# jonaselgammal/GPry

Measured on AMD Instinct MI355X. Metric: gp_refit_plus_nora_acq_cycle_throughput, higher is better.
Workload: dtype f64

## Files before the change

gpry_amd/_lib.py:

```python
import ctypes as C
import ctypes as _ct
import os

import numpy as np

_HERE = os.path.dirname(os.path.abspath(__file__))
LIB_PATH = os.path.join(_HERE, "libgpry_hip.so")

GPRY_MAX_DIM = 32
MASK_CLASSIFIED_INF = 1
MASK_OUTSIDE_TRUST = 2

KERNEL_IDS = {"rbf": 0, "matern12": 1, "matern32": 2, "matern52": 3}
KERNEL_WHITE = 0x10


class GpryAffine(C.Structure):
    _fields_ = [("has_x_affine", C.c_int),
                ("x_lo", C.c_double * GPRY_MAX_DIM),
                ("x_span", C.c_double * GPRY_MAX_DIM),
                ("y_mean", C.c_double), ("y_std", C.c_double),
                ("clip_hi", C.c_double)]


# ... 79 lines not shown
    "gpry_sweep_logexp": (C.c_int, [_vp, _vp, C.c_int64, _vp, C.c_double, C.c_double,
                                    C.c_double, _vp, _vp, _vp, _P(C.c_int64)]),
    "gpry_sweep_logexp_given": (C.c_int, [_vp, _vp, C.c_int64, _vp, _vp, _vp, C.c_double, C.c_double,
                                          C.c_double, _vp, _vp, _vp, _P(C.c_int64)]),
    "gpry_sweep_fetch": (C.c_int, [_vp, C.c_int64, _vp, _vp, _vp]),
    "gpry_sweep_prune_info": (C.c_int, [_vp, _vp, _vp]),
    "gpry_sweep_screen_info": (C.c_int, [_vp, _vp]),
    "gpry_sweep_topk": (C.c_int, [_vp, C.c_int64, _vp, C.c_int64, _vp, _P(C.c_int64),
                                  _P(C.c_double)]),
    "gpry_kb_reset": (C.c_int, [_vp]),
    "gpry_kb_register": (C.c_int, [_vp, _vp, C.c_int64, _P(C.c_int64), _vp]),
    "gpry_kb_gram": (C.c_int, [_vp, C.c_int64, _vp, _vp, _P(C.c_int64)]),
    "gpry_kb_gram_rows": (C.c_int, [_vp, _vp, C.c_int64, _vp, _vp, _P(C.c_int64)]),
    "gpry_kb_rank": (C.c_int, [_vp, _vp, C.c_int64, _vp, C.c_int64, _vp, _vp, _vp, _vp, C.c_int64, _vp, C.c_int64, _vp,
                               C.c_int64, _vp, _vp, _vp, _vp, _vp, _P(C.c_int64), _P(C.c_int64), _vp]),
    "gpry_comm_unique_id": (C.c_int, [_vp]),
    "gpry_comm_init": (C.c_int, [_vp, C.c_int, C.c_int, _vp, _P(_vp)]),
    "gpry_comm_destroy": (C.c_int, [_vp]),
    "gpry_comm_info": (C.c_int, [_vp, _P(C.c_int), _P(C.c_int), _P(C.c_int)]),
    "gpry_comm_allgather": (C.c_int, [_vp, _vp, C.c_int64, _vp]),
    "gpry_comm_allreduce_max": (C.c_int, [_vp, _vp, C.c_int64]),
    "gpry_comm_barrier": (C.c_int, [_vp]),
    "gpry_group_create": (C.c_int, [C.c_int, _P(C.c_int), _vp, _P(_vp)]),
    "gpry_group_destroy": (C.c_int, [_vp]),
    "gpry_group_size": (C.c_int, [_vp, _P(C.c_int), _P(C.c_int)]),
    "gpry_group_member": (_vp, [_vp, C.c_int]),
    "gpry_group_last_error": (C.c_char_p, [_vp]),
    "gpry_group_set_model": (C.c_int, [_vp, _vp, _vp, _vp, C.c_int64, C.c_int, C.c_int, _vp,
                                       _P(GpryAffine), _P(C.c_int)]),
    "gpry_group_set_gates": (C.c_int, [_vp, _vp, _vp, C.c_int64, C.c_double, C.c_double, C.c_int, _vp]),
# ... 819 lines not shown
        s_idx, s_y, s_sigma, s_acq, s_cond = slots
        for a, t in ((var0, np.float64), (idx, np.int64), (y, np.float64), (sigma, np.float64), (acq, np.float64),
                     (order, np.int64), (s_idx, np.int64), (s_y, np.float64), (s_sigma, np.float64),
                     (s_acq, np.float64), (s_cond, np.float64)):
            if a.dtype != t or not a.flags.c_contiguous:
                raise ValueError("kb_rank: arrays must be contiguous int64 / float64")
        if not (len(y) == len(sigma) == len(acq) == len(idx)) or len(params) != 5 or \
                not (len(s_idx) == len(s_y) == len(s_sigma) == len(s_acq) == len(s_cond)):
            raise ValueError("kb_rank: array lengths do not match")
        self._check(self._lib.gpry_kb_rank(self._h, _ptr(X_new), m_new, _ptr(var0), len(var0), _ptr(idx), _ptr(y),
                                           _ptr(sigma), _ptr(acq), len(idx), _ptr(order), len(order), _ptr(params),
                                           len(s_idx) - 1, _ptr(s_idx), _ptr(s_y), _ptr(s_sigma), _ptr(s_acq),
                                           _ptr(s_cond), C.byref(counter), C.byref(info), _ptr(stats)), "gpry_kb_rank")
        return counter.value, info.value, stats

    def timing_reset(self):
        self._check(self._lib.gpry_timing_reset(self._h), "gpry_timing_reset")

    def timing(self, name):
        ms, cnt = C.c_double(0.0), C.c_int64(0)
        self._lib.gpry_timing_get(self._h, name.encode(), C.byref(ms), C.byref(cnt))
        return ms.value, cnt.value

    def debug_gemm(self, A, B, C0, M, N, K, a_trans=False, b_trans=False, epi=0, kmode=0,
                   lower_only=False, tile_map=0):
        A, B = _f64(A), _f64(B)
        crow = (M + 127) // 128 if epi == 3 else M
        Cout = np.ascontiguousarray(np.zeros((crow, N)) if C0 is None else C0, dtype=np.float64).copy()
        self._check(self._lib.gpry_debug_gemm(self._h, _ptr(A), _ptr(B), _ptr(Cout), M, N, K,
                                              int(a_trans), int(b_trans), int(epi), int(kmode),
# ... 199 lines not shown
```

gpry_amd/csrc/api.hip:

```cpp
#include "sweep.h"
#include "kb_gram.h"
#include <algorithm>

int require_model(gpry_ctx* ctx, bool need_factor) {
    if (ctx->N <= 0) return gpry_fail(ctx, -1, "no training set (call gpry_set_train)");
    if (!ctx->have_theta) return gpry_fail(ctx, -1, "no hyperparameters (call gpry_set_theta)");
    if (need_factor && !ctx->factor_valid) return gpry_fail(ctx, -1, "model not factorised (call gpry_factorize)");
    if (need_factor && ctx->tf.has_x_affine)
        for (int k = 0; k < ctx->d; k++)
            if (!(ctx->tf.x_span[k] != 0.0) || !isfinite(ctx->tf.x_span[k]) || !isfinite(ctx->tf.x_lo[k]))
                return gpry_fail(ctx, -1, "affine map of X: span %g, offset %g in dimension %d of %d (gpry_set_affine of another model?)",
                                 ctx->tf.x_span[k], ctx->tf.x_lo[k], k, ctx->d);
    return 0;
}


static int copy_out_matrix(gpry_ctx* ctx, const double* dsrc, int64_t ld, int64_t rows, int64_t cols, double* hdst) {
    HIP_TRY(ctx, hipMemcpy2DAsync(hdst, sizeof(double) * cols, dsrc, sizeof(double) * ld,
                                  sizeof(double) * cols, rows, hipMemcpyDeviceToHost, ctx->stream));
    HIP_TRY(ctx, hipStreamSynchronize(ctx->stream));
    return 0;
}

bool panel_timed_out(int marker) { return (marker & 0xFF00) == 0x5A00; }
// ... 889 lines not shown
    for (int off = 32; off >= 1; off >>= 1) s += __shfl_xor(s, off);
    if (lane == 0) out[x] = C - s;
}

extern "C" {

int gpry_kb_reset(gpry_ctx* ctx) {
    if (!ctx) return gpry_fail(nullptr, -1, "gpry_kb_reset: ctx is NULL");
    GPRY_TRY(require_model(ctx, true));
    ctx->kb_n = 0;
    return 0;
}

int gpry_kb_register(gpry_ctx* ctx, const double* X, int64_t m, int64_t* first, double* var0) {
    if (!ctx) return gpry_fail(nullptr, -1, "gpry_kb_register: ctx is NULL");
    GPRY_TRY(serve_stop(ctx));
    GPRY_TRY(require_model(ctx, true));
    HIP_TRY(ctx, hipSetDevice(ctx->device));
    if (m <= 0) { if (first) *first = ctx->kb_n; return 0; }
    StageScope kb_scope(ctx, "kb_register");
    hipStream_t st = ctx->stream;
    const int64_t Np = ctx->Np;
    int64_t need = ctx->kb_n + round_up(m, 128);
    if (ctx->kb_n > 0 && ctx->kb_ld < Np) return gpry_fail(ctx, -4, "kb_register: session rows have stride %lld, model needs %lld", (long long)ctx->kb_ld, (long long)Np);
    if (need > ctx->kb_cap || Np > ctx->kb_ld) {
        int64_t cap = std::max<int64_t>(need, std::max<int64_t>(1024, need > ctx->kb_cap ? 2 * ctx->kb_cap : ctx->kb_cap));
        double *nU = nullptr, *nX = nullptr, *nO = nullptr;
        GPRY_TRY(dev_alloc(ctx, &nU, cap * Np));
        GPRY_TRY(dev_alloc(ctx, &nX, cap * ctx->dpad));
        GPRY_TRY(dev_alloc(ctx, &nO, 2 * cap));
        if (ctx->kb_n > 0) {
            HIP_TRY(ctx, hipMemcpyAsync(nU, ctx->dU, sizeof(double) * ctx->kb_n * Np, hipMemcpyDeviceToDevice, st));
            HIP_TRY(ctx, hipMemcpyAsync(nX, ctx->dXkb, sizeof(double) * ctx->kb_n * ctx->dpad, hipMemcpyDeviceToDevice, st));
        }
        HIP_TRY(ctx, hipStreamSynchronize(st));
        if (ctx->dU) GPRY_TRY(dev_free(ctx, ctx->dU));
        if (ctx->dXkb) GPRY_TRY(dev_free(ctx, ctx->dXkb));
        if (ctx->dkbout) GPRY_TRY(dev_free(ctx, ctx->dkbout));
        ctx->dU = nU; ctx->dXkb = nX; ctx->dkbout = nO; ctx->kb_cap = cap; ctx->kb_ld = Np;
    }
    const int64_t mp = round_up(m, 128);
    TmpBuf<double> bX, bpar;
    GPRY_TRY(bX.alloc(ctx, m * ctx->d));
    GPRY_TRY(bpar.alloc(ctx, 3 * GPRY_MAX_DIM));
    double *dX = bX.p, *dpar = bpar.p;
    HIP_TRY(ctx, hipMemcpyAsync(dX, X, sizeof(double) * m * ctx->d, hipMemcpyHostToDevice, st));
    double hpar[3 * GPRY_MAX_DIM];
    for (int k = 0; k < GPRY_MAX_DIM; k++) {
        hpar[k] = k < ctx->d ? ctx->tf.x_lo[k] : 0.0;
        hpar[GPRY_MAX_DIM + k] = k < ctx->d ? ctx->tf.x_span[k] : 1.0;
        hpar[2 * GPRY_MAX_DIM + k] = k < ctx->d ? exp(ctx->theta[1 + k]) : 1.0;
    }
    HIP_TRY(ctx, hipMemcpyAsync(dpar, hpar, sizeof(hpar), hipMemcpyHostToDevice, st));
    hipLaunchKernelGGL(scale_rows_kernel, dim3((unsigned)((m * ctx->dpad + 255) / 256)), dim3(256), 0, st, dX, m,
                       ctx->d, ctx->dpad, ctx->tf.has_x_affine, dpar, dpar + GPRY_MAX_DIM, dpar + 2 * GPRY_MAX_DIM,
                       ctx->dXkb + ctx->kb_n * ctx->dpad);
    GPRY_TRY(dev_grow(ctx, &ctx->dKst, &ctx->kst_cap, Np * mp));
    int64_t saveM = ctx->sw_M; ctx->sw_M = m;
    int rc = mp <= 512 ? launch_cross_build_small(ctx, dX, 0, mp, mp, ctx->dKst, nullptr, 1)
                       : launch_cross_build(ctx, dX, 0, mp, mp, ctx->dKst, nullptr, 1);
    ctx->sw_M = saveM;
// ... 1 lines not shown
    GemmArgs g = {};
    g.A = ctx->dKst; g.lda = mp;
    g.B = ctx->dV; g.ldb = Np;
    g.C = ctx->dU + ctx->kb_n * Np; g.ldc = Np;
    g.M = (int)mp; g.N = (int)Np; g.K = (int)Np;
    g.kmode = KM_B_UPPER; g.lower_only = 0; g.tile_map = TM_ROWMAJOR;
    {
        int ns = 1;
        while (ns < 8 && Np / (ns * 2) >= 256) ns *= 2;
        if (ns > 1) {
            GPRY_TRY(gemm_split_scratch(ctx, ns, mp * Np, &g.split_buf));
            g.nsplit = ns; g.split_stride = mp * Np;
        }
    }
    GPRY_TRY(gemm_f64_launch(ctx, g, true, true, EPI_STORE));
    if (var0) {
        hipLaunchKernelGGL(kb_var0_kernel, dim3((unsigned)((m + 3) / 4)), dim3(256), 0, st, ctx->dU, Np, ctx->kb_n, m,
                           Np, ctx_prior_var(ctx), ctx->dkbout);
        HIP_TRY(ctx, hipMemcpyAsync(var0, ctx->dkbout, sizeof(double) * m, hipMemcpyDeviceToHost, st));
    }
    HIP_TRY(ctx, hipStreamSynchronize(st));
    if (first) *first = ctx->kb_n;
    ctx->kb_n += m;
    return 0;
}

int gpry_kb_gram(gpry_ctx* ctx, int64_t p, double* G, double* kvec, int64_t* n) {
    if (!ctx) return gpry_fail(nullptr, -1, "gpry_kb_gram: ctx is NULL");
    GPRY_TRY(require_model(ctx, true));
    HIP_TRY(ctx, hipSetDevice(ctx->device));
    if (p < 0 || p >= ctx->kb_n) return gpry_fail(ctx, -1, "kb_gram: index %lld out of range [0, %lld)", (long long)p, (long long)ctx->kb_n);
    StageScope kb_scope(ctx, "kb_gram");
    hipStream_t st = ctx->stream;
    int64_t nn = ctx->kb_n;
    GPRY_TRY(ensure_pinned(ctx, (int64_t)sizeof(double) * 2 * nn));
    double* hres = static_cast<double*>(ctx->hpin);
    double* dres = static_cast<double*>(ctx->hpin_dev);
    hipLaunchKernelGGL(kb_gram_kernel, dim3((unsigned)((nn + 3) / 4)), dim3(256), 0, st, ctx->dU, ctx->Np, nn, p,
                       ctx->Np, ctx->dXkb, ctx->dpad, ctx->kernel_id, exp(ctx->theta[0]), dres, dres + nn);
    HIP_TRY(ctx, hipGetLastError());
// ... 76 lines not shown
```

gpry_amd/csrc/common.h:

```cpp
#pragma once
#include <hip/hip_runtime.h>
#include <stdint.h>
#include <stdio.h>
#include <string.h>
#include <math.h>
#include <string>
#include <vector>
#include <map>

#include "../../include/gpry_hip.h"

#define GPRY_THETA_MAX (2 + GPRY_MAX_DIM)
#define GPRY_BPAR_ROW (2 + GPRY_MAX_DIM)
#define GPRY_BPAR_WHITE (1 + GPRY_MAX_DIM)
#define GPRY_TILE 128
#define GPRY_NB 64

typedef double v4d __attribute__((ext_vector_type(4)));

struct StageTimer {
    double total_ms = 0.0;
    int64_t count = 0;
    std::vector<std::pair<hipEvent_t, hipEvent_t>> pending;
};
// ... 116 lines not shown
    unsigned long long* dsel = nullptr;
    enum { DSEL_NAN = 0,
           DSEL_STATE = 0,
           DSEL_EMIT = 4,
           DSEL_SURV = 6,
           DSEL_GIDX = 7,
           DSEL_LIVE = 8,
           DSEL_FALL = 9,
           DSEL_WORDS = 64 };

    int64_t kb_n = 0, kb_cap = 0;
    int64_t kb_ld = 0;
    double* dU = nullptr;
    double* dXkb = nullptr;
    double* dkbout = nullptr;

    double* dbord = nullptr;
    int64_t bord_cap = 0;
    int64_t n_border = 0;

    void* trtri_plan = nullptr;
    void* trtri_pipe = nullptr;
    int64_t opt_gemm_streamk = 5632;
    int64_t opt_topk_host = 16384;
    int opt_factor_pipeline = 1;
    int opt_factor_pipeline_min = 1280;
    void* chol_plan = nullptr;

    void* srv = nullptr;
    int opt_predict_serve = 1;
// ... 311 lines not shown
```

gpry_amd/csrc/ctx.hip:

```cpp
#include "common.h"
#include <string>
#include <stdarg.h>
#include <dlfcn.h>

thread_local char g_last_error[1024] = {0};
void trtri_plan_free(gpry_ctx* ctx);
void overlap_plan_free(gpry_ctx* ctx);

int gpry_fail(gpry_ctx* ctx, int code, const char* fmt, ...) {
    va_list ap;
    va_start(ap, fmt);
    vsnprintf(g_last_error, sizeof(g_last_error), fmt, ap);
    va_end(ap);
    if (ctx) { strncpy(ctx->err, g_last_error, sizeof(ctx->err) - 1); }
    return code;
}

template <typename T>
int dev_alloc(gpry_ctx* ctx, T** p, int64_t count) {
    *p = nullptr;
    if (count <= 0) count = 1;
    HIP_TRY(ctx, hipMalloc((void**)p, sizeof(T) * (size_t)count));
    return 0;
}
// ... 200 lines not shown
    (void)hipSetDevice(ctx->device);
    (void)hipStreamSynchronize(ctx->stream);
    if (ctx->stream2) (void)hipStreamSynchronize(ctx->stream2);
    timers_collect(ctx);
    serve_free(ctx);
    trtri_plan_free(ctx);
    trtri_pipe_free(ctx);
    overlap_plan_free(ctx);
    void* bufs[] = {ctx->dX, ctx->dXs, ctx->dy, ctx->dnoise, ctx->dA, ctx->dV, ctx->dW, ctx->dW2, ctx->dW3,
                    ctx->dalpha_, ctx->dvec, ctx->dinfo, ctx->dparams, ctx->dXc, ctx->dmask, ctx->dy_all,
                    ctx->dsig_all, ctx->dacq_all, ctx->dKst, ctx->dpart, ctx->dkeys, ctx->dhist, ctx->dselp,
                    ctx->dcand, ctx->dsel, ctx->dU, ctx->dXkb, ctx->dkbout, ctx->pr.dXc, ctx->pr.dmask,
                    ctx->pr.dy, ctx->pr.dsig, ctx->pr.dacq, ctx->dG,
                    ctx->gate_sv, ctx->gate_coef, ctx->gate_trust, ctx->dsplit, ctx->dbord, ctx->barena, ctx->dXcs, ctx->dYcs,
                    ctx->dub, ctx->dXg, ctx->dgidx, ctx->snap.dV, ctx->snap.dalpha_, ctx->snap.dXs, ctx->snap.dX, ctx->dmc, ctx->dknn,
                    ctx->dph, ctx->djoint, ctx->dloo, ctx->dsvm, ctx->dhess, ctx->dtg, ctx->dpw};
    for (void* b : bufs) if (b) (void)hipFree(b);
    if (ctx->hpin) (void)hipHostFree(ctx->hpin);
    if (ctx->hloo) (void)hipHostFree(ctx->hloo);
    if (ctx->hsvm) (void)hipHostFree(ctx->hsvm);
    if (ctx->hbres) (void)hipHostFree(ctx->hbres);
    (void)hipStreamDestroy(ctx->stream);
    if (ctx->stream2) (void)hipStreamDestroy(ctx->stream2);
    for (hipEvent_t ev : ctx->ev_pool) (void)hipEventDestroy(ev);
    for (hipStream_t st : ctx->tp_streams) (void)hipStreamDestroy(st);
    for (hipEvent_t ev : ctx->tp_events) (void)hipEventDestroy(ev);
    delete ctx;
    return 0;
}

const char* gpry_last_error(gpry_ctx* ctx) { return ctx ? ctx->err : g_last_error; }
// ... 44 lines not shown
    OPT_INT("sweep_upload", opt_sweep_upload, 0, 1, (void)0),
    OPT_INT("sweep_overlap", opt_sweep_overlap, 0, 1, (void)0),
    OPT_INT("sweep_prune", opt_sweep_prune, 0, 1, (void)0),
    OPT_INT("sweep_mean_bound", opt_sweep_mean_bound, 0, 1, (void)0),
    OPT_INT("sweep_screen", opt_sweep_screen, 0, 1, (void)0),
    OPT_INT("sweep_small_map", opt_sweep_small_map, 0, 1, (void)0),
    OPT_INT("select_fused", opt_select_fused, 0, 1, (void)0),
    OPT_INT("prune_one_select", opt_prune_one_select, 0, 1, (void)0),
    OPT_INT("chol_stacked", opt_chol_stacked, 0, BIG, c->lml_cache = false),
    OPT_INT("chol_stacked_dense", opt_chol_stacked_dense, 0, 1, c->lml_cache = false),
    OPT_INT("predict_gates", opt_predict_gates, 0, 1, (void)0),
    OPT_INT("predict_serve", opt_predict_serve, 0, 1, (void)0),
    OPT_INT("serve_idle_us", opt_serve_idle_us, 10, 1000000, (void)0),
    OPT_INT("mcmc_mapped", opt_mcmc_mapped, 0, 1, (void)0),
    OPT_INT("kb_rank", opt_kb_rank, 0, 1, (void)0),
    OPT_INT("svm_iters_per_launch", opt_svm_iters, 1, BIG, (void)0),
};
#undef OPT_INT
const OptionSpec* find_option(const char* key) {
    for (const OptionSpec& o : OPTIONS) if (!strcmp(o.key, key)) return &o;
    return nullptr;
}
}

int gpry_ctx_set_option(gpry_ctx* ctx, const char* key, int64_t value) {
    if (!ctx || !key) return gpry_fail(ctx, -1, "gpry_ctx_set_option: NULL argument");
    GPRY_TRY(serve_stop(ctx));
    const OptionSpec* o = find_option(key);
    if (!o) return gpry_fail(ctx, -1, "unknown option '%s'", key);
    if (value < o->lo || value > o->hi)
// ... 374 lines not shown
```

gpry_amd/csrc/kb_rank.hip:

```cpp
#include "common.h"
#include "kb_gram.h"
#include "kb_rank_core.h"
#include <memory>

#define KB_ROWS_MAX 64
struct KbRowList { int64_t p[KB_ROWS_MAX]; };

__global__ __launch_bounds__(256) void kb_gram_rows_kernel(const double* __restrict__ U, int64_t ldu, int64_t n, KbRowList rows,
                                                           int64_t Np, const double* __restrict__ Xkb, int dpad, int kid,
                                                           double C, double* __restrict__ out) {
    const int64_t x = (int64_t)blockIdx.x * 4 + (threadIdx.x >> 6);
    if (x >= n) return;
    double* o = out + (int64_t)blockIdx.y * 2 * n;
    kb_gram_entry(U, ldu, x, rows.p[blockIdx.y], Np, Xkb, dpad, kid, C, o, o + n);
}

namespace {
struct RowServer {
    gpry_ctx* ctx;
    int64_t nn;
    std::vector<const double*> G, kv;
    std::vector<std::unique_ptr<double[]>> store;
    int64_t launches = 0, rows = 0;

// ... 16 lines not shown
                               static_cast<double*>(ctx->hpin_dev));
            HIP_TRY(ctx, hipGetLastError());
            HIP_TRY(ctx, hipStreamSynchronize(ctx->stream));
            store.emplace_back(new double[(size_t)len]);
            double* blk = store.back().get();
            memcpy(blk, ctx->hpin, sizeof(double) * (size_t)len);
            for (int j = 0; j < cnt; j++) { G[rl.p[j]] = blk + (size_t)j * 2 * nn; kv[rl.p[j]] = blk + (size_t)j * 2 * nn + nn; }
            launches++; rows += cnt;
        }
        return 0;
    }
    static int fetch_cb(void* user, const int64_t* p, int n) { return static_cast<RowServer*>(user)->fetch(p, n); }
};
}

extern "C" {

int gpry_kb_gram_rows(gpry_ctx* ctx, const int64_t* p, int64_t n_rows, double* G, double* kvec, int64_t* n) {
    if (!ctx) return gpry_fail(nullptr, -1, "gpry_kb_gram_rows: ctx is NULL");
    GPRY_TRY(require_model(ctx, true));
    HIP_TRY(ctx, hipSetDevice(ctx->device));
    if (!p || !G || !kvec || n_rows <= 0 || n_rows > 16384) return gpry_fail(ctx, -1, "kb_gram_rows: bad arguments");
    if (ctx->kb_n <= 0) return gpry_fail(ctx, -1, "kb_gram_rows: no registered candidates");
    StageScope kb_scope(ctx, "kb_rank");
    RowServer rs{ctx, ctx->kb_n};
    rs.G.assign((size_t)rs.nn, nullptr); rs.kv.assign((size_t)rs.nn, nullptr);
    GPRY_TRY(rs.fetch(p, (int)n_rows));
    for (int64_t j = 0; j < n_rows; j++) {
        memcpy(G + j * rs.nn, rs.G[p[j]], sizeof(double) * rs.nn);
        memcpy(kvec + j * rs.nn, rs.kv[p[j]], sizeof(double) * rs.nn);
// ... 23 lines not shown
        if (ctx->kb_n + m_new != n_session)
            return gpry_fail(ctx, -1, "kb_rank: session has %lld candidates, %lld new rows, caller expects %lld",
                             (long long)ctx->kb_n, (long long)m_new, (long long)n_session);
        GPRY_TRY(gpry_kb_register(ctx, X_new, m_new, &first, var0 + (n_session - m_new)));
    }
    if (ctx->kb_n != n_session)
        return gpry_fail(ctx, -1, "kb_rank: session has %lld candidates, caller expects %lld", (long long)ctx->kb_n, (long long)n_session);
    for (int64_t i = 0; i < n_offer; i++)
        if (idx[i] < 0 || idx[i] >= n_session) return gpry_fail(ctx, -1, "kb_rank: offer %lld has session index %lld", (long long)i, (long long)idx[i]);
    for (int64_t k = 0; k < n_order; k++)
        if (order[k] < 0 || order[k] >= n_offer) return gpry_fail(ctx, -1, "kb_rank: order[%lld] = %lld", (long long)k, (long long)order[k]);
    const int n = (int)n_points;
    for (int t = 0; t <= n; t++)
        if (slot_idx[t] >= n_session || (slot_idx[t] < 0 && slot_acq_cond[t] > -INFINITY))
            return gpry_fail(ctx, -1, "kb_rank: slot %d has session index %lld", t, (long long)slot_idx[t]);
    StageScope kb_scope(ctx, "kb_rank");
    RowServer rs{ctx, n_session};
    rs.G.assign((size_t)n_session, nullptr); rs.kv.assign((size_t)n_session, nullptr);
    {
        std::vector<int64_t> spec;
        for (int t = 0; t < n; t++) if (slot_idx[t] >= 0 && slot_acq_cond[t] > -INFINITY) spec.push_back(slot_idx[t]);
        for (int64_t k = 0; k < n_order && k < 2 * (int64_t)n; k++) spec.push_back(idx[order[k]]);
        if (!spec.empty()) GPRY_TRY(rs.fetch(spec.data(), (int)spec.size()));
    }
    kb_rank::Params prm = {params[0], params[1], params[2], params[3], params[4]};
    kb_rank::Pool P = {n, slot_idx, slot_y, slot_sigma, slot_acq, slot_acq_cond, *cache_counter};
    kb_rank::Ranker rk(n, n_session, var0, prm, rs.G.data(), rs.kv.data(), &RowServer::fetch_cb, &rs, n_order + n + 1);
    const int64_t rc = rk.add(P, idx, y, sigma, acq, order, n_order);
    *cache_counter = P.cache_counter;
    if (stats) { stats[0] = rs.launches; stats[1] = rs.rows; stats[2] = rk.fetches(); }
    if (rc < 0) return ctx->err[0] ? (int)rc : gpry_fail(ctx, (int)rc, "kb_rank: the ranking failed (%lld)", (long long)rc);
    *info = rc;
    return 0;
}

}
```

gpry_amd/csrc/sweep.h:

```cpp
#pragma once
#include "common.h"

template <typename T>
struct TmpBuf {
    T* p = nullptr;
    TmpBuf() = default;
    TmpBuf(const TmpBuf&) = delete;
    TmpBuf& operator=(const TmpBuf&) = delete;
    ~TmpBuf() { if (p) (void)hipFree(p); }
    int alloc(gpry_ctx* ctx, int64_t count) { return dev_alloc(ctx, &p, count); }
};

static inline int ensure_part(gpry_ctx* ctx, int64_t need) { return dev_grow(ctx, &ctx->dpart, &ctx->part_cap, need); }

#define PRUNED_SIGMA (-1.0)

enum SweepKind {
    SWEEP_PREDICT,
    SWEEP_FULL,
    SWEEP_STAGE_A
};
struct SweepRequest {
    SweepKind kind = SWEEP_FULL;
    bool have_mask = false;
    bool want_std = true;
    bool y_given = false;
    double zeta = 0.0, baseline = 0.0, sigma_n = 0.0;
};
int run_sweep(gpry_ctx* ctx, int64_t M, const SweepRequest& rq);
int upload_candidates(gpry_ctx* ctx, const double* X, int64_t M, const uint8_t* mask, bool upload_later = false);
int launch_logexp(gpry_ctx* ctx, const double* mu, const double* sd, int64_t n, double zeta, double baseline, double sigma_n, double* acq);
int prune_eval(gpry_ctx* ctx, int64_t n);
int prune_complete(gpry_ctx* ctx);
```

gpry_amd/csrc/sweep.hip:

```cpp
#include "sweep.h"
#include "acq_math.h"
#include <algorithm>

__global__ void logexp_kernel(const double* __restrict__ mu, const double* __restrict__ sd, int64_t n, double zeta,
                              double baseline, double sigma_n, double* __restrict__ acq) {
    int64_t i = (int64_t)blockIdx.x * blockDim.x + threadIdx.x;
    if (i < n) acq[i] = logexp_value(mu[i], sd[i], zeta, baseline, sigma_n);
}
int launch_logexp(gpry_ctx* ctx, const double* mu, const double* sd, int64_t n, double zeta, double baseline, double sigma_n, double* acq) {
    hipLaunchKernelGGL(logexp_kernel, dim3((unsigned)((n + 255) / 256)), dim3(256), 0, ctx->stream, mu, sd, n, zeta, baseline, sigma_n, acq);
    HIP_TRY(ctx, hipGetLastError());
    return 0;
}

__device__ __forceinline__ double sum_partials(const double* __restrict__ part, int nt, int64_t ldp, int64_t col) {
    double s = 0.0;
#pragma unroll 8
    for (int t = 0; t < nt; t++) s += part[(int64_t)t * ldp + col];
    return s;
}
__device__ __forceinline__ double finish_y(double mu_, unsigned mk, const FinishParams& fp) {
    double y = mu_ * fp.y_std + fp.y_mean;
    y = fmin(y, fp.clip_hi);
    if (mk) y = -INFINITY;
// ... 94 lines not shown
        y_all[m] = finish_y(mu_, mask ? mask[m] : 0u, fp);
    }
    const double ss = sum_partials(ss_part, nt, ldp, i);
    const double sd = finish_sd(ss, mask ? mask[m] : 0u, fp);
    sig_all[m] = sd;
    acq_all[m] = logexp_value(y_all[m], sd, fp.zeta, fp.baseline, fp.sigma_n);
}

__global__ void gather_rows_kernel(const double* __restrict__ Xc, int d, const int64_t* __restrict__ gidx, int64_t n,
                                   int64_t n_pad, double* __restrict__ Xg) {
    int64_t e = (int64_t)blockIdx.x * blockDim.x + threadIdx.x;
    if (e >= n_pad * d) return;
    const int64_t i = e / d;
    const int k = (int)(e - i * d);
    Xg[e] = i < n ? Xc[gidx[i] * d + k] : 0.0;
}

template <int NS>
__global__ __launch_bounds__(1024) void splitk_sumsq_kernel(const double* __restrict__ P, int64_t stride,
                                                            int64_t ldp, double* __restrict__ ss_part) {
    __shared__ double red[16][64];
    const int ti = blockIdx.x, col = threadIdx.x & 63, rg = threadIdx.x >> 6;
    const int64_t c = (int64_t)blockIdx.y * 64 + col;
    double acc = 0.0;
#pragma unroll
    for (int rr = 0; rr < 8; rr += 2) {
        const int64_t off = ((int64_t)ti * 128 + rg * 8 + rr) * ldp + c;
        double v0[NS], v1[NS];
#pragma unroll
        for (int y = 0; y < NS; y++) { v0[y] = P[(int64_t)y * stride + off]; v1[y] = P[(int64_t)y * stride + off + ldp]; }
// ... 542 lines not shown
```

gpry_amd/gp_acquisition.py:

```python
import os
import inspect
import sys
import warnings
from collections.abc import Mapping
from copy import deepcopy
from functools import partial
from time import time

import numpy as np

import scipy.optimize

import gpry_amd.acquisition_functions as gpryacqfuncs
from gpry_amd.proposal import CentroidsProposer, PartialProposer, Proposer
from gpry_amd.tools import get_Xnumber, get_random_generator, is_in_bounds, remove_0_weight_samples


def builtin_names():
    return [name for name, obj in inspect.getmembers(sys.modules[__name__])
            if inspect.isclass(obj) and issubclass(obj, GenericGPAcquisition)
            and obj is not GenericGPAcquisition]


class NestedSamplerNotInstalledError(Exception):
# ... 679 lines not shown
            for row in self._X_already_proposed:
                hit = near[np.all(X_dev[near] == row, axis=1)] if near.size else near
                if hit.size:
                    exclude.append(int(hit[0]))
        exclude = np.unique(np.asarray(exclude, dtype=np.int64))
        self.acq_func_y_sigma = partial(self.acq_func.f, baseline=gpr.y_max,
                                        noise_level=gpr.noise_level, zeta=self.acq_func.zeta)
        self.log(f"({(time() - t_start):.2g} sec) " +
                 (f"Obtained new MC sample with {self.sampler}" if resample
                  else "Re-evaluated previous MC sample"), level=2)
        t_rank = time()
        self.pool = RankedPool(n_points, gpr=gpr, acq_func=self.acq_func_y_sigma,
                               verbose=self.verbose - 3)
        K = int(self.shortlist_size or max(256, 16 * n_points))
        fed = 0
        with np.errstate(divide="ignore"):
            while True:
                top, bound, exhausted = self._shortlist(gpr, K, exclude)
                new = top[fed:]
                if len(new):
                    self.pool.add(X_dev[new["idx"]], new["y"].copy(), new["sigma"].copy(),
                                  new["acq"].copy(), method="single sort acq")
                fed = len(top)
                if exhausted or self.pool.min_acq >= bound:
                    break
                K *= 4
        self.stats.update(shortlist=fed, cache_models=self.pool.cache_counter,
                          rank_s=time() - t_rank, rank_native=self.pool.rank_native)
        pruned_on = getattr(self, "_pruned_on", [])
        if pruned_on:
            self.stats["prune"] = [t.sweep_prune_info() for t in pruned_on]
            for t, st in zip(pruned_on, self.stats["prune"]):
                if hasattr(t, "sweep_screen_info"):
                    st["certified"] = t.sweep_screen_info()["certified"]
        else:
# ... 112 lines not shown
    def _add_native(self, X, y, sigma, acq):
        gpr = self._gpr
        dev = getattr(gpr, "device", None)
        if dev is None or not hasattr(dev, "kb_rank") or not hasattr(gpr, "kb_session"):
            return False
        if gpr.infinities_classifier is not None or np.iterable(gpr.noise_level) or not 0 < len(X) <= 16384:
            return False
        params = self._native_params()
        if params is None or not dev.get_option("kb_rank"):
            return False
        y, sigma, acq = (np.ascontiguousarray(a, dtype=np.float64) for a in (y, sigma, acq))
        if np.isnan(acq).any():
            return False
        sess = gpr.kb_session()
        filled = self.acq_cond > -np.inf
        s_idx = np.array([sess._index.get(np.ascontiguousarray(row, dtype=float).tobytes(), -1) for row in self.X],
                         dtype=np.int64)
        if np.any(s_idx[filled] < 0):
            return False
        order = np.ascontiguousarray(np.argsort(acq)[::-1], dtype=np.int64)
        slots = (s_idx, self.y, self.sigma, self.acq, self.acq_cond)
        _, (models, info, stats) = sess.rank(X, y, sigma, acq, order, params, slots)
        self.cache_counter += models
        held = s_idx >= 0
        self.X[held] = sess.X[s_idx[held]]
        self.X[~held] = 0.0
        self.gpr_cond = _LazyModels(sess, s_idx, int(np.count_nonzero(self.acq_cond[:-1] > -np.inf)))
        self.rank_stats = tuple(int(v) for v in stats)
        if info:
            raise np.linalg.LinAlgError(
                f"{info}-th appended point makes the augmented kernel matrix non positive "
                "definite. Try gradually increasing the 'noise_level' parameter of your "
                "GaussianProcessRegressor estimator.")
        return True

    def add_bulk(self, X, y, sigma, acq, i_start=0):
        X, y, sigma, acq = np.atleast_2d(X), np.asarray(y), np.asarray(sigma), np.asarray(acq)
        slot = i_start
        while True:
            if slot == 0:
                a_cond = acq
            else:
                model = self.cache_model(slot - 1)
                a_cond = self._acq_func(y, model.predict_std(X, validate=False))
            if a_cond.size == 0:
                return
            best = int(np.argmax(a_cond))
            if a_cond[best] == np.inf:
                return
# ... 96 lines not shown
```

gpry_amd/kriging.py:

```python
import copy

import numpy as np

from gpry_amd import _lib


class KBSession:

    def __init__(self, gpr):
        self.gpr = gpr
        self.dev = gpr.device
        gpr._push_affine()
        self.dev.kb_reset()
        d = gpr.d
        self.X = np.empty((0, d))
        self.var0 = np.empty(0)
        self.masked = np.empty(0, bool)
        self._index = {}
        self._gram = {}
        self._last_cond = None
        kid, full = gpr._device_theta()
        self.C = float(np.exp(full[0]))
        self.white = float(np.exp(full[-1])) if kid & _lib.KERNEL_WHITE else None
        self.std_y = gpr._y_affine()[1]

    @property
    def n(self):
        return len(self.var0)

    def _assign(self, X):
        X = np.ascontiguousarray(np.atleast_2d(X), dtype=float)
        idx = np.empty(len(X), dtype=np.int64)
        new_rows = []
        for i, row in enumerate(X):
            key = row.tobytes()
            j = self._index.get(key)
            if j is None:
                j = self.n + len(new_rows)
                self._index[key] = j
                new_rows.append(row)
            idx[i] = j
        return idx, (np.array(new_rows) if new_rows else None)

    def _commit(self, Xn, var0):
        self.X = np.vstack([self.X, Xn])
        self.var0 = np.append(self.var0, var0)
        clf = self.gpr.infinities_classifier
        if clf is None:
            m = np.zeros(len(Xn), bool)
        else:
            Xn_ = np.ascontiguousarray(self.gpr.preprocessing_X.transform(Xn))
            m = np.logical_not(clf.predict(Xn_, validate=False))
        self.masked = np.append(self.masked, m)

    def register(self, X):
        idx, Xn = self._assign(X)
        if Xn is not None:
            first, var0 = self.dev.kb_register(Xn)
            if first != self.n:
                raise _lib.GpryHipError("KB session out of sync with the device")
            self._commit(Xn, var0)
        return idx

    def rank(self, X, y, sigma, acq, order, params, slots):
        idx, Xn = self._assign(X)
        m_new = 0 if Xn is None else len(Xn)
        var0 = np.concatenate([self.var0, np.empty(m_new)])
        try:
# ... 113 lines not shown
```

include/gpry_hip.h:

```cpp
#ifndef GPRY_HIP_H
#define GPRY_HIP_H

#include <stdint.h>

#ifdef __cplusplus
extern "C" {
#endif

typedef struct gpry_ctx gpry_ctx;
typedef struct gpry_comm gpry_comm;
typedef struct gpry_group gpry_group;

enum { GPRY_RBF = 0, GPRY_MATERN12 = 1, GPRY_MATERN32 = 2, GPRY_MATERN52 = 3 };
#define GPRY_KERNEL_WHITE 0x10

#define GPRY_MAX_DIM 32

typedef struct {
    int has_x_affine;
    double x_lo[GPRY_MAX_DIM];
    double x_span[GPRY_MAX_DIM];
    double y_mean, y_std;
    double clip_hi;
} gpry_affine;
// ... 161 lines not shown
int gpry_sweep_topk(gpry_ctx* ctx, int64_t Kp, const int64_t* exclude, int64_t n_exclude,
                    gpry_cand* top, int64_t* n_out, double* bound);
int gpry_sweep_prune_info(gpry_ctx* ctx, int64_t* info, double* dinfo);
int gpry_sweep_screen_info(gpry_ctx* ctx, int64_t out[2]);

int gpry_kb_reset(gpry_ctx* ctx);
int gpry_kb_register(gpry_ctx* ctx, const double* X, int64_t m, int64_t* first,
                     double* var0);
int gpry_kb_gram(gpry_ctx* ctx, int64_t p, double* G, double* kvec, int64_t* n);
int gpry_kb_gram_rows(gpry_ctx* ctx, const int64_t* p, int64_t n_rows, double* G, double* kvec, int64_t* n);
int gpry_kb_rank(gpry_ctx* ctx, const double* X_new, int64_t m_new, double* var0, int64_t n_session,
                 const int64_t* idx, const double* y, const double* sigma, const double* acq, int64_t n_offer,
                 const int64_t* order, int64_t n_order, const double* params, int64_t n_points,
                 int64_t* slot_idx, double* slot_y, double* slot_sigma, double* slot_acq, double* slot_acq_cond,
                 int64_t* cache_counter, int64_t* info, int64_t* stats);

int gpry_comm_unique_id(uint8_t id[128]);
int gpry_comm_init(gpry_ctx* ctx, int world, int rank, const uint8_t id[128],
                   gpry_comm** out);
int gpry_comm_destroy(gpry_comm* comm);
int gpry_comm_info(gpry_comm* comm, int* world, int* rank, int* device);
int gpry_comm_allgather(gpry_comm* comm, const void* send, int64_t bytes, void* recv);
int gpry_comm_allreduce_max(gpry_comm* comm, double* inout, int64_t n);
int gpry_comm_barrier(gpry_comm* comm);

int gpry_group_create(int n, const int* devices, gpry_ctx* adopt0, gpry_group** out);
int gpry_group_destroy(gpry_group* group);
int gpry_group_size(gpry_group* group, int* n, int* transport);
gpry_ctx* gpry_group_member(gpry_group* group, int i);
const char* gpry_group_last_error(gpry_group* group);
// ... 36 lines not shown
```

Measured before the change: 68.41 million.

## Fuse shortlist top-k, pool-row registration and ranking into one native tail call

Adds a native gpry_multi_add_tail entry point that runs the sweep top-k, gathers the chosen candidate rows on the device from the resident pool instead of copying them from the host, registers them into the kriging-believer session, and ranks them in a single call. The prior var0 is written into mapped pinned memory so the register step skips its own synchronisation, and the rank's first fetch absorbs it. It is meant to remove Python round trips, host-to-device copies of X and extra stream syncs in the first acquisition pass. The cost is a more complex path with several fallbacks (ties, NaNs, non-empty session, grouped or multi-rank sweeps) and a lazily built session index.

New measurement: 68.03 million. Within noise of the previous version (-0.5%).

```diff
diff --git a/gpry_amd/_lib.py b/gpry_amd/_lib.py
--- a/gpry_amd/_lib.py
+++ b/gpry_amd/_lib.py
@@ -117,6 +117,8 @@
     "gpry_kb_gram_rows": (C.c_int, [_vp, _vp, C.c_int64, _vp, _vp, _P(C.c_int64)]),
     "gpry_kb_rank": (C.c_int, [_vp, _vp, C.c_int64, _vp, C.c_int64, _vp, _vp, _vp, _vp, C.c_int64, _vp, C.c_int64, _vp,
                                C.c_int64, _vp, _vp, _vp, _vp, _vp, _P(C.c_int64), _P(C.c_int64), _vp]),
+    "gpry_multi_add_tail": (C.c_int, [_vp, C.c_int64, _vp, C.c_int64, _vp, C.c_int64, _vp, _P(C.c_int64), _P(C.c_double), _vp,
+                                      _vp, _vp, _vp, _vp, _vp, _P(C.c_int64), _P(C.c_int64), _vp]),
     "gpry_comm_unique_id": (C.c_int, [_vp]),
     "gpry_comm_init": (C.c_int, [_vp, C.c_int, C.c_int, _vp, _P(_vp)]),
     "gpry_comm_destroy": (C.c_int, [_vp]),
@@ -966,6 +968,34 @@
                                            _ptr(s_cond), C.byref(counter), C.byref(info), _ptr(stats)), "gpry_kb_rank")
         return counter.value, info.value, stats
 
+    MULTI_ADD_TAIL_NOT_TAKEN, MULTI_ADD_TAIL_SHORTLIST, MULTI_ADD_TAIL_RANKED = 0, 1, 2
+
+    def multi_add_tail(self, K, exclude, params, slots):
+        K = int(K)
+        top = np.zeros(max(K, 1), dtype=CAND_DTYPE)
+        var0 = np.empty(max(K, 1))
+        n_out, bound = C.c_int64(0), C.c_double(0.0)
+        if exclude is not None and len(exclude):
+            exclude = np.ascontiguousarray(np.sort(np.asarray(exclude, dtype=np.int64)))
+            nex = len(exclude)
+        else:
+            exclude, nex = None, 0
+        params = _f64(params)
+        s_idx, s_y, s_sigma, s_acq, s_cond = slots
+        for a, t in ((s_idx, np.int64), (s_y, np.float64), (s_sigma, np.float64), (s_acq, np.float64), (s_cond, np.float64)):
+            if a.dtype != t or not a.flags.c_contiguous or len(a) != len(s_idx):
+                raise ValueError("multi_add_tail: the slots must be contiguous int64 / float64 arrays of one length")
+        if len(params) != 5:
+            raise ValueError("multi_add_tail: five parameters")
+        counter, info = C.c_int64(0), C.c_int64(0)
+        stats = np.zeros(6, dtype=np.int64)
+        self._check(self._lib.gpry_multi_add_tail(self._h, K, _ptr(exclude), nex, _ptr(params), len(s_idx) - 1, _ptr(top),
+                                                  C.byref(n_out), C.byref(bound), _ptr(var0), _ptr(s_idx), _ptr(s_y),
+                                                  _ptr(s_sigma), _ptr(s_acq), _ptr(s_cond), C.byref(counter),
+                                                  C.byref(info), _ptr(stats)), "gpry_multi_add_tail")
+        n = n_out.value
+        return int(stats[0]), top[:n], bound.value, var0[:n], counter.value, info.value, stats
+
     def timing_reset(self):
         self._check(self._lib.gpry_timing_reset(self._h), "gpry_timing_reset")
 
diff --git a/gpry_amd/csrc/api.hip b/gpry_amd/csrc/api.hip
--- a/gpry_amd/csrc/api.hip
+++ b/gpry_amd/csrc/api.hip
@@ -927,10 +927,23 @@
 
 int gpry_kb_register(gpry_ctx* ctx, const double* X, int64_t m, int64_t* first, double* var0) {
     if (!ctx) return gpry_fail(nullptr, -1, "gpry_kb_register: ctx is NULL");
+    return kb_register_rows(ctx, X, nullptr, m, first, var0, nullptr);
+}
+
+}
+
+int kb_register_rows(gpry_ctx* ctx, const double* X, const int64_t* pool_idx, int64_t m, int64_t* first, double* var0,
+                     double* var0_mapped) {
     GPRY_TRY(serve_stop(ctx));
     GPRY_TRY(require_model(ctx, true));
     HIP_TRY(ctx, hipSetDevice(ctx->device));
     if (m <= 0) { if (first) *first = ctx->kb_n; return 0; }
+    if (pool_idx) {
+        if (!ctx->dXc || ctx->sw_M <= 0) return gpry_fail(ctx, -1, "kb_register: no candidate pool resident");
+        for (int64_t i = 0; i < m; i++)
+            if (pool_idx[i] < 0 || pool_idx[i] >= ctx->sw_M)
+                return gpry_fail(ctx, -1, "kb_register: pool index %lld out of range [0, %lld)", (long long)pool_idx[i], (long long)ctx->sw_M);
+    }
     StageScope kb_scope(ctx, "kb_register");
     hipStream_t st = ctx->stream;
     const int64_t Np = ctx->Np;
@@ -954,10 +967,21 @@
     }
     const int64_t mp = round_up(m, 128);
     TmpBuf<double> bX, bpar;
-    GPRY_TRY(bX.alloc(ctx, m * ctx->d));
-    GPRY_TRY(bpar.alloc(ctx, 3 * GPRY_MAX_DIM));
-    double *dX = bX.p, *dpar = bpar.p;
-    HIP_TRY(ctx, hipMemcpyAsync(dX, X, sizeof(double) * m * ctx->d, hipMemcpyHostToDevice, st));
+    double *dX = nullptr, *dpar = nullptr;
+    if (pool_idx) {
+        const int64_t need_s = 3 * GPRY_MAX_DIM + m + m * ctx->d;
+        GPRY_TRY(dev_grow(ctx, &ctx->dkbstage, &ctx->kbstage_cap, round_up(need_s, 4096)));
+        dpar = ctx->dkbstage;
+        int64_t* didx = reinterpret_cast<int64_t*>(ctx->dkbstage + 3 * GPRY_MAX_DIM);
+        dX = ctx->dkbstage + 3 * GPRY_MAX_DIM + m;
+        HIP_TRY(ctx, hipMemcpyAsync(didx, pool_idx, sizeof(int64_t) * m, hipMemcpyHostToDevice, st));
+        GPRY_TRY(gather_pool_rows(ctx, didx, m, dX));
+    } else {
+        GPRY_TRY(bX.alloc(ctx, m * ctx->d));
+        GPRY_TRY(bpar.alloc(ctx, 3 * GPRY_MAX_DIM));
+        dX = bX.p; dpar = bpar.p;
+        HIP_TRY(ctx, hipMemcpyAsync(dX, X, sizeof(double) * m * ctx->d, hipMemcpyHostToDevice, st));
+    }
     double hpar[3 * GPRY_MAX_DIM];
     for (int k = 0; k < GPRY_MAX_DIM; k++) {
         hpar[k] = k < ctx->d ? ctx->tf.x_lo[k] : 0.0;
@@ -989,16 +1013,19 @@
         }
     }
     GPRY_TRY(gemm_f64_launch(ctx, g, true, true, EPI_STORE));
-    if (var0) {
+    if (var0 || var0_mapped) {
         hipLaunchKernelGGL(kb_var0_kernel, dim3((unsigned)((m + 3) / 4)), dim3(256), 0, st, ctx->dU, Np, ctx->kb_n, m,
-                           Np, ctx_prior_var(ctx), ctx->dkbout);
-        HIP_TRY(ctx, hipMemcpyAsync(var0, ctx->dkbout, sizeof(double) * m, hipMemcpyDeviceToHost, st));
-    }
-    HIP_TRY(ctx, hipStreamSynchronize(st));
+                           Np, ctx_prior_var(ctx), var0_mapped ? var0_mapped : ctx->dkbout);
+        HIP_TRY(ctx, hipGetLastError());
+        if (!var0_mapped) HIP_TRY(ctx, hipMemcpyAsync(var0, ctx->dkbout, sizeof(double) * m, hipMemcpyDeviceToHost, st));
+    }
+    if (!var0_mapped) HIP_TRY(ctx, hipStreamSynchronize(st));
     if (first) *first = ctx->kb_n;
     ctx->kb_n += m;
     return 0;
 }
+
+extern "C" {
 
 int gpry_kb_gram(gpry_ctx* ctx, int64_t p, double* G, double* kvec, int64_t* n) {
     if (!ctx) return gpry_fail(nullptr, -1, "gpry_kb_gram: ctx is NULL");
diff --git a/gpry_amd/csrc/common.h b/gpry_amd/csrc/common.h
--- a/gpry_amd/csrc/common.h
+++ b/gpry_amd/csrc/common.h
@@ -154,6 +154,9 @@
     double* dU = nullptr;
     double* dXkb = nullptr;
     double* dkbout = nullptr;
+    double* dkbstage = nullptr;
+    int64_t kbstage_cap = 0;
+    int opt_multi_add_tail = 1;
 
     double* dbord = nullptr;
     int64_t bord_cap = 0;
diff --git a/gpry_amd/csrc/ctx.hip b/gpry_amd/csrc/ctx.hip
--- a/gpry_amd/csrc/ctx.hip
+++ b/gpry_amd/csrc/ctx.hip
@@ -238,7 +238,7 @@
                     ctx->pr.dy, ctx->pr.dsig, ctx->pr.dacq, ctx->dG,
                     ctx->gate_sv, ctx->gate_coef, ctx->gate_trust, ctx->dsplit, ctx->dbord, ctx->barena, ctx->dXcs, ctx->dYcs,
                     ctx->dub, ctx->dXg, ctx->dgidx, ctx->snap.dV, ctx->snap.dalpha_, ctx->snap.dXs, ctx->snap.dX, ctx->dmc, ctx->dknn,
-                    ctx->dph, ctx->djoint, ctx->dloo, ctx->dsvm, ctx->dhess, ctx->dtg, ctx->dpw};
+                    ctx->dph, ctx->djoint, ctx->dloo, ctx->dsvm, ctx->dhess, ctx->dtg, ctx->dpw, ctx->dkbstage};
     for (void* b : bufs) if (b) (void)hipFree(b);
     if (ctx->hpin) (void)hipHostFree(ctx->hpin);
     if (ctx->hloo) (void)hipHostFree(ctx->hloo);
@@ -313,6 +313,7 @@
     OPT_INT("serve_idle_us", opt_serve_idle_us, 10, 1000000, (void)0),
     OPT_INT("mcmc_mapped", opt_mcmc_mapped, 0, 1, (void)0),
     OPT_INT("kb_rank", opt_kb_rank, 0, 1, (void)0),
+    OPT_INT("multi_add_tail", opt_multi_add_tail, 0, 1, (void)0),
     OPT_INT("svm_iters_per_launch", opt_svm_iters, 1, BIG, (void)0),
 };
 #undef OPT_INT
diff --git a/gpry_amd/csrc/kb_rank.hip b/gpry_amd/csrc/kb_rank.hip
--- a/gpry_amd/csrc/kb_rank.hip
+++ b/gpry_amd/csrc/kb_rank.hip
@@ -1,4 +1,4 @@
-#include "common.h"
+#include "sweep.h"
 #include "kb_gram.h"
 #include "kb_rank_core.h"
 #include <memory>
@@ -54,6 +54,11 @@
 };
 }
 
+static int rank_offer(gpry_ctx* ctx, double* var0, int64_t n_session, const int64_t* idx, const double* y, const double* sigma,
+                      const double* acq, const int64_t* order, int64_t n_order, const double* params, int n,
+                      int64_t* slot_idx, double* slot_y, double* slot_sigma, double* slot_acq, double* slot_acq_cond,
+                      int64_t* cache_counter, int64_t* info, int64_t* stats, const double* var0_late, int64_t n_late);
+
 extern "C" {
 
 int gpry_kb_gram_rows(gpry_ctx* ctx, const int64_t* p, int64_t n_rows, double* G, double* kvec, int64_t* n) {
@@ -107,6 +112,16 @@
     for (int t = 0; t <= n; t++)
         if (slot_idx[t] >= n_session || (slot_idx[t] < 0 && slot_acq_cond[t] > -INFINITY))
             return gpry_fail(ctx, -1, "kb_rank: slot %d has session index %lld", t, (long long)slot_idx[t]);
+    return rank_offer(ctx, var0, n_session, idx, y, sigma, acq, order, n_order, params, n, slot_idx, slot_y, slot_sigma, slot_acq,
+                      slot_acq_cond, cache_counter, info, stats, nullptr, 0);
+}
+
+}
+
+static int rank_offer(gpry_ctx* ctx, double* var0, int64_t n_session, const int64_t* idx, const double* y, const double* sigma,
+                      const double* acq, const int64_t* order, int64_t n_order, const double* params, int n,
+                      int64_t* slot_idx, double* slot_y, double* slot_sigma, double* slot_acq, double* slot_acq_cond,
+                      int64_t* cache_counter, int64_t* info, int64_t* stats, const double* var0_late, int64_t n_late) {
     StageScope kb_scope(ctx, "kb_rank");
     RowServer rs{ctx, n_session};
     rs.G.assign((size_t)n_session, nullptr); rs.kv.assign((size_t)n_session, nullptr);
@@ -115,7 +130,9 @@
         for (int t = 0; t < n; t++) if (slot_idx[t] >= 0 && slot_acq_cond[t] > -INFINITY) spec.push_back(slot_idx[t]);
         for (int64_t k = 0; k < n_order && k < 2 * (int64_t)n; k++) spec.push_back(idx[order[k]]);
         if (!spec.empty()) GPRY_TRY(rs.fetch(spec.data(), (int)spec.size()));
+        else if (var0_late) HIP_TRY(ctx, hipStreamSynchronize(ctx->stream));
     }
+    if (var0_late) memcpy(var0 + (n_session - n_late), var0_late, sizeof(double) * (size_t)n_late);
     kb_rank::Params prm = {params[0], params[1], params[2], params[3], params[4]};
     kb_rank::Pool P = {n, slot_idx, slot_y, slot_sigma, slot_acq, slot_acq_cond, *cache_counter};
     kb_rank::Ranker rk(n, n_session, var0, prm, rs.G.data(), rs.kv.data(), &RowServer::fetch_cb, &rs, n_order + n + 1);
@@ -127,4 +144,46 @@
     return 0;
 }
 
+extern "C" int gpry_multi_add_tail(gpry_ctx* ctx, int64_t K, const int64_t* exclude, int64_t n_exclude, const double* params,
+                                   int64_t n_points, gpry_cand* top, int64_t* n_out, double* bound, double* var0,
+                                   int64_t* slot_idx, double* slot_y, double* slot_sigma, double* slot_acq, double* slot_acq_cond,
+                                   int64_t* cache_counter, int64_t* info, int64_t* stats) {
+    if (!ctx) return gpry_fail(nullptr, -1, "gpry_multi_add_tail: ctx is NULL");
+    GPRY_TRY(require_model(ctx, true));
+    HIP_TRY(ctx, hipSetDevice(ctx->device));
+    if (!params || !top || !n_out || !bound || !var0 || !slot_idx || !slot_y || !slot_sigma || !slot_acq || !slot_acq_cond ||
+        !cache_counter || !info || !stats)
+        return gpry_fail(ctx, -1, "multi_add_tail: NULL argument");
+    if (n_exclude > 0 && !exclude) return gpry_fail(ctx, -1, "multi_add_tail: n_exclude > 0 but exclude is NULL");
+    if (n_points < 1 || n_points > 4096 || K < 1) return gpry_fail(ctx, -1, "multi_add_tail: bad sizes (n_points %lld, K %lld)", (long long)n_points, (long long)K);
+    for (int k = 0; k < 6; k++) stats[k] = 0;
+    *info = 0; *n_out = 0;
+    if (!ctx->opt_multi_add_tail || !ctx->opt_kb_rank || !ctx->sw_pruned || ctx->sw_M <= 0 || ctx->kb_n != 0 || K > 16384) return 0;
+    for (int t = 0; t <= (int)n_points; t++)
+        if (slot_idx[t] >= 0 || slot_acq_cond[t] > -INFINITY) return gpry_fail(ctx, -1, "multi_add_tail: the pool must be empty");
+    GPRY_TRY(gpry_sweep_topk(ctx, K, exclude, n_exclude, top, n_out, bound));
+    stats[0] = 1;
+    const int64_t m = *n_out;
+    if (m <= 0) return 0;
+    for (int64_t i = 0; i < m; i++) if (top[i].acq != top[i].acq) return 0;
+    for (int64_t i = 1; i < m; i++) if (top[i].acq == top[i - 1].acq) return 0;
+    std::vector<int64_t> pool_idx((size_t)m), ident((size_t)m);
+    std::vector<double> y((size_t)m), sigma((size_t)m), acq((size_t)m);
+    for (int64_t i = 0; i < m; i++) {
+        pool_idx[(size_t)i] = top[i].idx; ident[(size_t)i] = i;
+        y[(size_t)i] = top[i].y; sigma[(size_t)i] = top[i].sigma; acq[(size_t)i] = top[i].acq;
+    }
+    const int64_t off = 2 * m * KB_ROWS_MAX;
+    GPRY_TRY(ensure_pinned(ctx, (int64_t)sizeof(double) * (off + m)));
+    int64_t first = -1;
+    GPRY_TRY(kb_register_rows(ctx, nullptr, pool_idx.data(), m, &first, nullptr, static_cast<double*>(ctx->hpin_dev) + off));
+    if (first != 0 || ctx->kb_n != m) return gpry_fail(ctx, -4, "multi_add_tail: session out of step (first %lld, rows %lld)", (long long)first, (long long)ctx->kb_n);
+    stats[4] = m;
+    int64_t rstats[3] = {0, 0, 0};
+    GPRY_TRY(rank_offer(ctx, var0, m, ident.data(), y.data(), sigma.data(), acq.data(), ident.data(), m, params, (int)n_points,
+                        slot_idx, slot_y, slot_sigma, slot_acq, slot_acq_cond, cache_counter, info, rstats,
+                        static_cast<const double*>(ctx->hpin) + off, m));
+    stats[0] = 2;
+    stats[1] = rstats[0]; stats[2] = rstats[1]; stats[3] = rstats[2];
+    return 0;
 }
diff --git a/gpry_amd/csrc/sweep.h b/gpry_amd/csrc/sweep.h
--- a/gpry_amd/csrc/sweep.h
+++ b/gpry_amd/csrc/sweep.h
@@ -32,3 +32,6 @@
 int launch_logexp(gpry_ctx* ctx, const double* mu, const double* sd, int64_t n, double zeta, double baseline, double sigma_n, double* acq);
 int prune_eval(gpry_ctx* ctx, int64_t n);
 int prune_complete(gpry_ctx* ctx);
+int gather_pool_rows(gpry_ctx* ctx, const int64_t* didx, int64_t n, double* out);
+int kb_register_rows(gpry_ctx* ctx, const double* X, const int64_t* pool_idx, int64_t m, int64_t* first, double* var0,
+                     double* var0_mapped);
diff --git a/gpry_amd/csrc/sweep.hip b/gpry_amd/csrc/sweep.hip
--- a/gpry_amd/csrc/sweep.hip
+++ b/gpry_amd/csrc/sweep.hip
@@ -132,6 +132,14 @@
     const int64_t i = e / d;
     const int k = (int)(e - i * d);
     Xg[e] = i < n ? Xc[gidx[i] * d + k] : 0.0;
+}
+
+int gather_pool_rows(gpry_ctx* ctx, const int64_t* didx, int64_t n, double* out) {
+    if (n <= 0) return 0;
+    hipLaunchKernelGGL(gather_rows_kernel, dim3((unsigned)((n * ctx->d + 255) / 256)), dim3(256), 0, ctx->stream, ctx->dXc, ctx->d,
+                       didx, n, n, out);
+    HIP_TRY(ctx, hipGetLastError());
+    return 0;
 }
 
 template <int NS>
diff --git a/gpry_amd/gp_acquisition.py b/gpry_amd/gp_acquisition.py
--- a/gpry_amd/gp_acquisition.py
+++ b/gpry_amd/gp_acquisition.py
@@ -717,11 +717,24 @@
                                verbose=self.verbose - 3)
         K = int(self.shortlist_size or max(256, 16 * n_points))
         fed = 0
+        first = None
+        if (not getattr(self, "_sweep_grouped", False) and (self.comm is None or self.comm.world == 1)
+                and self._sweep_lo == 0 and self._sweep_dev is getattr(gpr, "device", None)
+                and len(getattr(self, "_pruned_on", [])) == 1 and self._pruned_on[0] is self._sweep_dev
+                and getattr(self, "_lazy", None) is not None):
+            first = self.pool.add_tail_native(K, exclude, X_dev)
+        self.stats["tail_native"] = first is not None
         with np.errstate(divide="ignore"):
             while True:
-                top, bound, exhausted = self._shortlist(gpr, K, exclude)
+                ranked = False
+                if first is not None:
+                    (top, bound, ranked), first = first, None
+                    top = top.copy()
+                    exhausted = len(top) < K
+                else:
+                    top, bound, exhausted = self._shortlist(gpr, K, exclude)
                 new = top[fed:]
-                if len(new):
+                if len(new) and not ranked:
                     self.pool.add(X_dev[new["idx"]], new["y"].copy(), new["sigma"].copy(),
                                   new["acq"].copy(), method="single sort acq")
                 fed = len(top)
@@ -864,13 +877,16 @@
             return False
         sess = gpr.kb_session()
         filled = self.acq_cond > -np.inf
-        s_idx = np.array([sess._index.get(np.ascontiguousarray(row, dtype=float).tobytes(), -1) for row in self.X],
-                         dtype=np.int64)
+        s_idx = np.array([sess.index_of(row) for row in self.X], dtype=np.int64)
         if np.any(s_idx[filled] < 0):
             return False
         order = np.ascontiguousarray(np.argsort(acq)[::-1], dtype=np.int64)
         slots = (s_idx, self.y, self.sigma, self.acq, self.acq_cond)
         _, (models, info, stats) = sess.rank(X, y, sigma, acq, order, params, slots)
+        self._finish_native(sess, s_idx, models, info, stats)
+        return True
+
+    def _finish_native(self, sess, s_idx, models, info, stats):
         self.cache_counter += models
         held = s_idx >= 0
         self.X[held] = sess.X[s_idx[held]]
@@ -882,7 +898,39 @@
                 f"{info}-th appended point makes the augmented kernel matrix non positive "
                 "definite. Try gradually increasing the 'noise_level' parameter of your "
                 "GaussianProcessRegressor estimator.")
-        return True
+
+    def add_tail_native(self, K, exclude, X_pool):
+        gpr = self._gpr
+        dev = getattr(gpr, "device", None)
+        if dev is None or not hasattr(dev, "multi_add_tail") or not hasattr(dev, "kb_rank") or not hasattr(gpr, "kb_session"):
+            return None
+        if gpr.infinities_classifier is not None or np.iterable(gpr.noise_level) or not 0 < K <= 16384:
+            return None
+        params = self._native_params()
+        if params is None or not dev.get_option("kb_rank") or not dev.get_option("multi_add_tail"):
+            return None
+        if np.any(self.acq_cond > -np.inf):
+            return None
+        sess = gpr.kb_session()
+        if sess.n:
+            return None
+        s_idx = np.full(len(self.y), -1, dtype=np.int64)
+        slots = (s_idx, self.y, self.sigma, self.acq, self.acq_cond)
+        try:
+            state, top, bound, var0, models, info, stats = dev.multi_add_tail(
+                K, exclude, [params["sigma_n"], sess.noise_alpha(), params["baseline"], params["zeta"], sess.std_y], slots)
+        except Exception:
+            gpr._kb = None
+            raise
+        self.tail_stats = tuple(int(v) for v in stats)
+        if state == dev.MULTI_ADD_TAIL_NOT_TAKEN:
+            return None
+        if state != dev.MULTI_ADD_TAIL_RANKED:
+            return top, bound, False
+        sess.adopt(X_pool[top["idx"]], var0)
+        self.rank_native = True
+        self._finish_native(sess, s_idx, models, info, stats[1:4])
+        return top, bound, True
 
     def add_bulk(self, X, y, sigma, acq, i_start=0):
         X, y, sigma, acq = np.atleast_2d(X), np.asarray(y), np.asarray(sigma), np.asarray(acq)
diff --git a/gpry_amd/kriging.py b/gpry_amd/kriging.py
--- a/gpry_amd/kriging.py
+++ b/gpry_amd/kriging.py
@@ -17,6 +17,7 @@
         self.var0 = np.empty(0)
         self.masked = np.empty(0, bool)
         self._index = {}
+        self._indexed = 0
         self._gram = {}
         self._last_cond = None
         kid, full = gpr._device_theta()
@@ -28,7 +29,24 @@
     def n(self):
         return len(self.var0)
 
+    def _fill_index(self):
+        for j in range(self._indexed, self.n):
+            self._index.setdefault(self.X[j].tobytes(), j)
+        self._indexed = self.n
+
+    def index_of(self, row):
+        self._fill_index()
+        return self._index.get(np.ascontiguousarray(row, dtype=float).tobytes(), -1)
+
+    def adopt(self, X, var0):
+        if self.gpr.infinities_classifier is not None:
+            raise ValueError("KBSession.adopt: not with an infinities classifier")
+        self.X = np.vstack([self.X, np.ascontiguousarray(X, dtype=float)])
+        self.var0 = np.append(self.var0, var0)
+        self.masked = np.append(self.masked, np.zeros(len(var0), bool))
+
     def _assign(self, X):
+        self._fill_index()
         X = np.ascontiguousarray(np.atleast_2d(X), dtype=float)
         idx = np.empty(len(X), dtype=np.int64)
         new_rows = []
@@ -52,6 +70,7 @@
             Xn_ = np.ascontiguousarray(self.gpr.preprocessing_X.transform(Xn))
             m = np.logical_not(clf.predict(Xn_, validate=False))
         self.masked = np.append(self.masked, m)
+        self._indexed = self.n
 
     def register(self, X):
         idx, Xn = self._assign(X)
diff --git a/include/gpry_hip.h b/include/gpry_hip.h
--- a/include/gpry_hip.h
+++ b/include/gpry_hip.h
@@ -199,6 +199,10 @@
                  const int64_t* order, int64_t n_order, const double* params, int64_t n_points,
                  int64_t* slot_idx, double* slot_y, double* slot_sigma, double* slot_acq, double* slot_acq_cond,
                  int64_t* cache_counter, int64_t* info, int64_t* stats);
+int gpry_multi_add_tail(gpry_ctx* ctx, int64_t K, const int64_t* exclude, int64_t n_exclude, const double* params,
+                        int64_t n_points, gpry_cand* top, int64_t* n_out, double* bound, double* var0,
+                        int64_t* slot_idx, double* slot_y, double* slot_sigma, double* slot_acq, double* slot_acq_cond,
+                        int64_t* cache_counter, int64_t* info, int64_t* stats);
 
 int gpry_comm_unique_id(uint8_t id[128]);
 int gpry_comm_init(gpry_ctx* ctx, int world, int rank, const uint8_t id[128],
```
